# pzimbrod/fem-glass-tempering

Measured on AMD Instinct MI355X. Metric: DOF-updates/sec (coupled thermo-visco time step, 3D CG1 hex), higher is better.
Workload: dtype f64; 1 GPU; C4 3D plate CG1/CG1 400x400x50 hex (8200851 T-dofs), dt 0.1, coupled 6-term Prony; parallelism=single GPU, one partition (no communication), output=none (reference writes VTX/XDMF every step), krylov_form=PETSc KSPCG, geometric-multigrid V-cycle preconditioner, preconditioner=gmg, visco_fields=state (T, Tf, Tf_partial, phi, xi, s_tilde, sigma_tilde, sigma)

## Files before the change

fem-glass-tempering_amd/csrc/tv_cg.hip:

```cpp
#include <algorithm>
#include <cstdlib>

#include "tv_stencil.h"


#include <cstdio>
#include <vector>

namespace tv {
namespace {


using buf_t = __amdgpu_buffer_rsrc_t;
using b64v = unsigned int __attribute__((ext_vector_type(2)));
constexpr uint32_t kBadOff = 0x40000000u;
__device__ __forceinline__ buf_t mk_rsrc(const void* p, uint32_t bytes) {
  const uint64_t a = (uint64_t)p;
  const uint32_t lo = __builtin_amdgcn_readfirstlane((uint32_t)a);
  const uint32_t hi = __builtin_amdgcn_readfirstlane((uint32_t)(a >> 32));
  void* q = (void*)(((uint64_t)hi << 32) | lo);
  return __builtin_amdgcn_make_buffer_rsrc(q, (short)0, (int)__builtin_amdgcn_readfirstlane(bytes), 0x00020000);
}
__device__ __forceinline__ double bload(buf_t r, uint32_t off) {
  return __builtin_bit_cast(double, __builtin_amdgcn_raw_buffer_load_b64(r, (int)off, 0, 0));
// ... 771 lines not shown
    const double us_p = My0 * x0 + My1 * x1 + My2 * x2;
    const double vs_p = Ky0 * x0 + Ky1 * x1 + Ky2 * x2;
    double um_p = us_p;
    if (MODE == MODE_RES) um_p = My0 * lds[NA - 1][buf][wave][lane] + My1 * vm + My2 * lds[NA - 1][buf][wave + 2][lane];
    const double t_p = um_p + da * vs_p;
    if (L >= q0 + 1 && L <= q1) {
      const int q = L - 1;
      const double2* cq = cql[q - q0 + 1];
      const double2 c01 = cq[0], c23 = cq[1], c45 = cq[2], c67 = cq[3], c89 = cq[4];
      const double S1 = c01.x * t_m + c01.y * t_c + c23.x * t_p + (c23.y * us_m + c45.x * us_c + c45.y * us_p);
      const double S2 = c67.x * us_m + c67.y * us_c + c89.x * us_p;
      const double2 xlo = cxl[0][lane], xdi = cxl[1][lane], xup = cxl[2][lane];
      const double Lt = xup.x * S1 + xup.y * S2;
      const double Rt = xlo.x * S1 + xlo.y * S2;
      const double y = (xdi.x * S1 + xdi.y * S2) + (shr1(Lt) + shl1(Rt));
      const bool q_owned = (raxis == 2) ? true : (q >= kb && q < ke);
      const bool q_inwin = (raxis == 2) ? true : (q >= wb && q < we);
      const bool wr = writer && row_ok && row_owned && q_owned;
      const bool inwin = row_inwin && q_inwin;
      double yb = y;
      if (fq0 && q == 0) yb += yq0;
      if (fq1 && q == nQ - 1) yb += yq1;
      if (POST) {
        const double xm = xdi.x, xk = xdi.y;
        const double dI = xm * My1 * c01.y + ((xk * My1 * c67.y + xm * Ky1 * c67.y) + xm * My1 * c45.x);
        const double dq = (bnd_lr || bnd_q(q)) ? pd : 1.0 / dI;
        const double zq = xc + pa.omega * dq * (pr - yb);
        bstore(rso, inwin ? vo_wr + plane_off(q) : kBadOff, zq);
        zz += wr ? zq * zq : 0.0;
        zr += wr ? zq * pr : 0.0;
      } else {
        bstore(rso, inwin ? vo_wr + plane_off(q) : kBadOff, yb);
      }
      if (MODE == MODE_JAC && !POST) dot += wr ? xc * yb : 0.0;
    }
    xc = x1;
    us_m = us_c; us_c = us_p;
    t_m = t_c; t_c = t_p;
  };
  for (int L = q0 - 1; L <= q1; L += PF + 1) {
#pragma unroll
    for (int s = 0; s <= PF; ++s) {
      const int sf = (s + PF) % (PF + 1);
      fetch(vo_own, L + s + PF, ra0[sf], ra1[sf]);
      fetch(vo_halo, L + s + PF, rh0[sf], rh1[sf]);
      fetch_post(L + s + PF, rr[sf], rd[sf]);
      step(L + s, ra0[s], ra1[s], rh0[s], rh1[s], POST ? rr[s] : 0.0, POST ? rd[s] : 0.0);
    }
  }
  if (POST) {
    zz = wave_sum(zz);
    zr = wave_sum(zr);
    if (lane == 0) {
      red[wave] = zz;
      fsm[wave] = zr;
    }
    __syncthreads();
    if (threadIdx.x == 0) {
      double a = 0.0, c = 0.0;
#pragma unroll
      for (int w = 0; w < R; ++w) {
        a += red[w];
        c += fsm[w];
      }
      store_partial(&partials[2 * (int64_t)bid], a);
      store_partial(&partials[2 * (int64_t)bid + 1], c);
    }
    return;
  }
  if (MODE == MODE_JAC && partials != nullptr) {
    dot = wave_sum(dot);
    if (lane == 0) red[wave] = dot;
    __syncthreads();
    if (threadIdx.x == 0) {
      double s = 0.0;
#pragma unroll
      for (int w = 0; w < R; ++w) s += red[w];
      store_partial(&partials[blockIdx.x], s);
    }
    fused_reduce_tail<1>(rt, nrec);
  }
}


__device__ __forceinline__ uint32_t ff_off_x(const CgGrid& g, int i, int j, int k) {
  const int f = (i == 0) ? 0 : (i == g.n0 - 1 ? 1 : -1);
  if (f < 0 || g.ffoff[f] < 0) return kBadOff;
  return (uint32_t)(g.ffoff[f] + j + (int64_t)g.n1 * k) * 8u;
}
__device__ __forceinline__ uint32_t ff_off_r(const CgGrid& g, int ra, int i, int j, int k) {
  const int c = (ra == 1) ? j : k, n = (ra == 1) ? g.n1 : g.n2;
  const int side = (c == 0) ? 0 : (c == n - 1 ? 1 : -1);
  if (side < 0 || i < 0 || i >= g.n0) return kBadOff;
  const int f = 2 * ra + side;
  if (g.ffoff[f] < 0) return kBadOff;
  return (uint32_t)(g.ffoff[f] + i + (int64_t)g.n0 * ((ra == 1) ? k : j)) * 8u;
}

struct CgsScal {
  double a, b;
  bool first;
};

template <bool INIT>
__device__ __forceinline__ void cgs_node(const CgsScal& k, double R, double S, double W, double D, double ff,
                                         double& s, double& r, double& u) {
  if (INIT) {
    s = 0.0;
    r = R;
  } else {
    const double wf = W + ff;
    s = k.first ? wf : wf + k.b * S;
    r = R - k.a * s;
  }
  u = D * r;
}

template <bool INIT, int R>
__device__ void face_block_cgs(const CgGrid& g, const CgsBuffers& v, const CgsScal& ks, int raxis,
                               double* __restrict__ partials, int fb, const FaceOff& fo, double* sm,
                               double (*red)[R]) {
  double (*sT)[kWave] = reinterpret_cast<double (*)[kWave]>(sm);
  double (*sP)[kWave] = reinterpret_cast<double (*)[kWave]>(sm + (R + 1) * kWave);
  double (*sCD)[R][kWave] = reinterpret_cast<double (*)[R][kWave]>(sm + 2 * (R + 1) * kWave);
  int f = 0;
  while (f < 5 && fb >= fo.off[f + 1]) ++f;
  const int a = f >> 1, side = f & 1;
  const int t1 = (a == 0) ? 1 : 0, t2 = (a == 2) ? 1 : 2;
  const int n[3] = {g.n0, g.n1, g.n2};
  const int n1 = n[t1], n2 = n[t2];
  const int nseg1 = (n1 + kSeg - 1) / kSeg;
  const int tile = fb - fo.off[f];
  const int seg = tile % nseg1, tb = tile / nseg1;
  const int lane = threadIdx.x & (kWave - 1);
  const int wave = __builtin_amdgcn_readfirstlane(threadIdx.x >> 6);
  const int c1 = seg * kSeg - 1 + lane;
  const int r0 = tb * (R - 1);
  const bool ok1 = c1 >= 0 && c1 < n1;
  const buf_t rsFin = mk_rsrc(v.fin, (uint32_t)(g.ffsize * 8));
  struct Stg {
    double tt, R_, D, S, W, fx, fr;
    bool ok;
  };
  auto stage_ld = [&](int cc2) -> Stg {
    Stg q{};
    q.ok = ok1 && cc2 >= 0 && cc2 < n2;
    int c[3];
    c[t1] = q.ok ? c1 : 0;
    c[t2] = q.ok ? cc2 : 0;
    c[a] = side ? n[a] - 1 : 0;
    const int64_t o = c[0] + (int64_t)g.n0 * c[1] + (int64_t)g.n0 * g.n1 * c[2];
    q.tt = v.T[o];
    q.R_ = v.rin[o];
    q.D = v.dinv[o];
    if (!INIT) {
      q.S = ks.first ? 0.0 : v.sin[o];
      q.W = v.win[o];
      q.fx = bload(rsFin, ff_off_x(g, c[0], c[1], c[2]));
      q.fr = bload(rsFin, ff_off_r(g, raxis, c[0], c[1], c[2]));
    }
    return q;
  };
  auto stage_st = [&](int row, const Stg& q) {
    double s, r, u;
    cgs_node<INIT>(ks, q.R_, q.S, q.W, q.D, INIT ? 0.0 : q.fx + q.fr, s, r, u);
    sT[row][lane] = q.ok ? q.tt : 0.0;
// ... 392 lines not shown
    const int nn[3] = {g.n0, g.n1, g.n2};
    double acc = 0.0;
#pragma unroll 1
    for (int a = 0; a < 3; ++a) {
      if ((c[a] == 0 && g.bnd[a][0]) || (c[a] == nn[a] - 1 && g.bnd[a][1]))
        acc += facet_direct<MODE, false>(g, i, j, k, a, T, x, nullptr, 0.0, true);
    }
    out[n] += acc;
    if (MODE == MODE_JAC) dot += x[n] * acc;
    if (MODE == MODE_RES && dinv != nullptr) dinv[n] = 1.0 / diag_value<3, true>(g, T, n);
  }
  if (MODE == MODE_JAC && partials != nullptr) {
    dot = wave_sum(dot);
    const int lane = threadIdx.x & 63, wave = threadIdx.x >> 6;
    if (lane == 0) red[wave] = dot;
    __syncthreads();
    if (threadIdx.x == 0) store_partial(&partials[blockIdx.x], (red[0] + red[1]) + (red[2] + red[3]));
  }
}


int dim_of(const CgGrid& g) { return g.deg2 ? 1 : (g.deg1 ? 2 : 3); }

constexpr int kMarchMinBlocks = 1024;
constexpr int kMarchMinQ = 6;
constexpr int kMarchSmallTiles = 256;

struct Launch {
  int blocks, nseg, kfirst, nplanes, wmode, rows;
  int nparts;
  bool march;
  int raxis, qchunk;
};

bool use_march(const CgGrid& g) {
  const int64_t bytes = (int64_t)g.n0 * g.n1 * g.n2 * 8;
  return dim_of(g) == 3 && bytes < (int64_t)kBadOff;
}

int bnd_blocks(const CgGrid& g) {
  int64_t b = (g.n_bnodes + kBlock - 1) / kBlock;
  return (int)std::max<int64_t>(1, std::min<int64_t>(b, 1024));
}

Launch plan(const CgGrid& g, bool ghosts) {
  Launch L{};
  L.nseg = (g.n0 + kSeg - 1) / kSeg;
  L.march = use_march(g);
  if (L.march) {
    L.raxis = (g.n2 >= g.n1) ? 2 : 1;
    L.rows = kRows;
    const int nR = (L.raxis == 1) ? g.n1 : g.n2;
    const int nQ = (L.raxis == 1) ? g.n2 : g.n1;
    const int nrb = (nR + L.rows - 1) / L.rows;
    int nchunks = 1;
    while ((int64_t)L.nseg * nrb * nchunks < kMarchMinBlocks && nQ / (nchunks * 2) >= kMarchMinQ) nchunks *= 2;
    while ((int64_t)L.nseg * nrb * nchunks < kMarchSmallTiles && nQ / (nchunks * 2) >= 2) nchunks *= 2;
    while ((nQ + nchunks - 1) / nchunks > kFaceChunk) ++nchunks;
    L.qchunk = (nQ + nchunks - 1) / nchunks;
    nchunks = (nQ + L.qchunk - 1) / L.qchunk;
    L.blocks = L.nseg * nrb * nchunks;
    L.nparts = L.blocks + face_offsets(g, L.rows, 3 - L.raxis).off[6];
    return L;
  }
  L.kfirst = ghosts ? g.k_begin - g.g_lo : g.k_begin;
  L.nplanes = (g.k_end - g.k_begin) + (ghosts ? g.g_lo + g.g_hi : 0);
  L.wmode = (g.n1 >= 4) ? 0 : 1;
  if (L.wmode == 0) {
    L.blocks = L.nseg * ((g.n1 + 3) / 4) * L.nplanes;
  } else {
    const int64_t waves = (int64_t)L.nseg * g.n1 * L.nplanes;
    L.blocks = (int)((waves + 3) / 4);
  }
  L.nparts = L.blocks;
  return L;
}

template <int MODE, bool FUSEP>
bool launch_rows(const CgGrid& g, const double* T, const double* in0, const double* in1, double* out,
                 double* pout, const PcgState* st, double* partials, bool ghosts, hipStream_t s,
                 const RedTail* tail = nullptr, int it_host = 0, bool addfaces = true, double* dinv_bnd = nullptr) {
  const Launch L = plan(g, ghosts);
  if (L.blocks <= 0) return false;
  if (L.march) {
    const bool folded = MODE == MODE_JAC;
    RedTail rt{};
    if (folded && tail && partials) rt = *tail;
    const FaceOff fo = folded ? face_offsets(g, L.rows, 3 - L.raxis) : FaceOff{};
    const int grid = L.blocks + fo.off[6];
    hipLaunchKernelGGL((k_cg_march<MODE, FUSEP, kRows, 1, 2>), dim3(grid), dim3(kRows * kWave), 0, s, g, T, in0, in1,
                       out, pout, st, partials, L.nseg, L.raxis, L.qchunk, rt, L.nparts, L.blocks, fo, it_host,
                       PostArgs{});
    if (folded && !FUSEP && addfaces && fo.off[6] > 0) {
      const int64_t nodes = 2 * ((int64_t)g.n1 * (g.w_end - g.w_begin) + (int64_t)g.n0 * std::max(g.n1, g.n2));
      const int nb = (int)std::max<int64_t>(1, std::min<int64_t>((nodes + kBlock - 1) / kBlock, 1024));
      hipLaunchKernelGGL(k_cg_addfaces, dim3(nb), dim3(kBlock), 0, s, g, out, L.raxis, st);
    }
    if (folded) return rt.counter != nullptr;
    if (g.n_bnodes > 0) {
      hipLaunchKernelGGL((k_cg_boundary<MODE, FUSEP>), dim3(bnd_blocks(g)), dim3(kBlock), 0, s, g, g.bnodes,
                         g.n_bnodes, T, FUSEP ? in1 : in0, pout, out, st,
                         partials ? partials + L.blocks : nullptr, dinv_bnd);
    }
    return false;
  }
  switch (dim_of(g)) {
    case 1:
      hipLaunchKernelGGL((k_cg_rows<1, MODE, FUSEP>), dim3(L.blocks), dim3(kBlock), 0, s, g, T, in0, in1, out,
                         pout, st, partials, L.nseg, L.kfirst, L.nplanes, L.wmode);
      break;
    case 2:
      hipLaunchKernelGGL((k_cg_rows<2, MODE, FUSEP>), dim3(L.blocks), dim3(kBlock), 0, s, g, T, in0, in1, out,
                         pout, st, partials, L.nseg, L.kfirst, L.nplanes, L.wmode);
      break;
    default:
      hipLaunchKernelGGL((k_cg_rows<3, MODE, FUSEP>), dim3(L.blocks), dim3(kBlock), 0, s, g, T, in0, in1, out,
                         pout, st, partials, L.nseg, L.kfirst, L.nplanes, L.wmode);
  }
  return false;
}

__global__ __launch_bounds__(kBlock) void k_mg_post_faces(FaceAdd fa, int raxis, const double* __restrict__ r,
                                                         const double* __restrict__ dinv, double omega,
                                                         double* __restrict__ z, double* __restrict__ partials,
                                                         int rec0, RedTail rt, const PcgState* __restrict__ st, int kb,
                                                         int ke, int wb, int we) {
  if (st->done) return;
  const int n0 = fa.n0, n1 = fa.n1, n2 = fa.n2;
  const int64_t nA = 2 * (int64_t)n1 * n2;
  const int nO = (raxis == 2) ? n1 : n2;
  const int64_t nB = 2 * (int64_t)(n0 - 2) * nO;
  double a0 = 0.0, a1 = 0.0;
  const FaceRsrc fr = face_rsrc(fa);
  for (int64_t t = blockIdx.x * (int64_t)kBlock + threadIdx.x; t < nA + nB; t += (int64_t)gridDim.x * kBlock) {
    int i, j, k;
    if (t < nA) {
      const int64_t pl = (int64_t)n1 * n2;
      const int side = (int)(t / pl);
      const int64_t e = t - side * pl;
      i = side ? n0 - 1 : 0;
      j = (int)(e % n1);
      k = (int)(e / n1);
    } else {
      const int64_t u = t - nA, pl = (int64_t)(n0 - 2) * nO;
      const int side = (int)(u / pl);
      const int64_t e = u - side * pl;
      i = 1 + (int)(e % (n0 - 2));
      const int o = (int)(e / (n0 - 2));
      if (raxis == 2) {
        j = o;
        k = side ? n2 - 1 : 0;
      } else {
        k = o;
        j = side ? n1 - 1 : 0;
      }
    }
    if (k < wb || k >= we) continue;
    const int64_t q = i + (int64_t)n0 * (j + (int64_t)n1 * k);
    const double zo = z[q], dq = dinv[q], rq = r[q];
    const double add = face_at_nb(fa, fr, i, j, k);
    const double zn = zo - omega * dq * add;
    z[q] = zn;
    if (k < kb || k >= ke) continue;
    a0 += zn * zn - zo * zo;
    a1 += (zn - zo) * rq;
  }
// ... 4 lines not shown
  if (lane == 0) {
    red[0][wave] = a0;
    red[1][wave] = a1;
  }
  __syncthreads();
  if (threadIdx.x < 2) {
    const int w = threadIdx.x;
    store_partial(&partials[2 * ((int64_t)rec0 + blockIdx.x) + w], (red[w][0] + red[w][1]) + (red[w][2] + red[w][3]));
  }
  fused_reduce_tail<2>(rt, rec0 + (int)gridDim.x);
}

__global__ __launch_bounds__(kBlock) void k_mg_prep_inject(MgPrep p) {
  const int64_t t = blockIdx.x * (int64_t)kBlock + threadIdx.x;
  int l = 0;
  while (l + 1 < p.nlev && t >= p.off_n[l + 1]) ++l;
  l = __builtin_amdgcn_readfirstlane(l);
  const MgXfer& x = p.xf[l];
  const int64_t e = t - p.off_n[l];
  const int64_t nc = (int64_t)x.cn[0] * x.cn[1] * x.cn[2];
  if (e >= nc) return;
  int c0 = (int)(e % x.cn[0]);
  int c1 = (int)((e / x.cn[0]) % x.cn[1]);
  int c2 = (int)(e / ((int64_t)x.cn[0] * x.cn[1]));
  for (int m = l; m >= 0; --m) {
    const MgXfer& y = p.xf[m];
    c0 = y.ri[0][3 * c0 + 1];
    c1 = y.ri[1][3 * c1 + 1];
    c2 = y.ri[2][3 * c2 + 1];
  }
  const MgXfer& b = p.xf[0];
  p.T[l][e] = p.Tbase[c0 + (int64_t)b.fn[0] * (c1 + (int64_t)b.fn[1] * c2)];
}

__global__ __launch_bounds__(kBlock) void k_mg_prep_diag(MgPrep p) {
  const int64_t t = blockIdx.x * (int64_t)kBlock + threadIdx.x;
  int l = 0;
  while (l + 1 < p.nlev && t >= p.off_b[l + 1]) ++l;
  l = __builtin_amdgcn_readfirstlane(l);
  const CgGrid& g = p.g[l];
  const int64_t e = t - p.off_b[l];
  if (e >= g.n_bnodes) return;
  const int64_t n = g.bnodes[e];
  p.dinv[l][n] = 1.0 / diag_value<3, true>(g, p.T[l], n);
}


template <int R>
__global__ __launch_bounds__(R * kWave) void k_cg_faces_all(CgGrid g, const double* __restrict__ T,
                                                            const double* __restrict__ x, FaceOff fo,
                                                            const PcgState* __restrict__ st) {
  if (st != nullptr && st->done) return;
  __shared__ double fsm[(8 * R + 8) * kWave];
  __shared__ double red[R];
  face_block<false, R>(g, T, x, x, x, 0.0, nullptr, RedTail{}, 0, (int)blockIdx.x, fo, fsm, red, 0);
}

}

int launch_cg_japply_post(const CgGrid& g, const double* T, const double* x, const double* r, const double* dinv,
                          double omega, double* z, const PcgState* st, double* partials, const RedTail* tail,
                          hipStream_t s) {
  const Launch L = plan(g, false);
  if (!L.march || g.n0 < 3) return -1;
  const FaceOff fo = face_offsets(g, L.rows, 3 - L.raxis);
  const int grid = L.blocks + fo.off[6];
  const PostArgs pa{r, dinv, omega};
  hipLaunchKernelGGL((k_cg_march<MODE_JAC, false, 8, 1, 2, true>), dim3(grid), dim3(8 * kWave), 0, s, g, T, x,
                     nullptr, z, nullptr, st, partials, L.nseg, L.raxis, L.qchunk, RedTail{}, L.nparts, L.blocks, fo,
                     0, pa);
  const FaceAdd fa = cg_face_add(g, 0);
  const int nO = (L.raxis == 2) ? g.n1 : g.n2;
  const int64_t nodes = 2 * (int64_t)g.n1 * g.n2 + 2 * (int64_t)(g.n0 - 2) * nO;
  constexpr int cap = 240;
  const int nb = (int)std::max<int64_t>(1, std::min<int64_t>((nodes + kBlock - 1) / kBlock, cap));
  const RedTail rt = tail ? *tail : RedTail{};
  hipLaunchKernelGGL(k_mg_post_faces, dim3(nb), dim3(kBlock), 0, s, fa, L.raxis, r, dinv, omega, z, partials,
                     L.blocks, rt, st, g.k_begin, g.k_end, g.w_begin, g.w_end);
  return L.blocks + nb;
}

bool cg_uses_march(const CgGrid& g) { return use_march(g); }

void launch_mg_prepare(const MgPrep& p, hipStream_t s) {
  const int64_t nn = p.off_n[p.nlev], nb = p.off_b[p.nlev];
  if (nn > 0) hipLaunchKernelGGL(k_mg_prep_inject, dim3((unsigned)((nn + kBlock - 1) / kBlock)), dim3(kBlock), 0, s, p);
  if (nb > 0) hipLaunchKernelGGL(k_mg_prep_diag, dim3((unsigned)((nb + kBlock - 1) / kBlock)), dim3(kBlock), 0, s, p);
}

int cg_num_blocks(const CgGrid& g, bool with_ghost_planes) { return plan(g, with_ghost_planes).nparts; }

FaceAdd cg_face_add(const CgGrid& g, int64_t t_off) {
  FaceAdd fa{};
  if (!use_march(g)) return fa;
  fa.on = 1;
  fa.n0 = g.n0;
  fa.n1 = g.n1;
  fa.n2 = g.n2;
  fa.t_off = t_off;
  fa.inv_n0 = 1.0 / g.n0;
  fa.inv_plane = 1.0 / ((double)g.n0 * g.n1);
  const int qaxis = 3 - plan(g, true).raxis;
  for (int f = 0; f < 6; ++f) fa.ff[f] = ((f >> 1) == qaxis) ? nullptr : g.fface[f];
  return fa;
}

void launch_cg_residual(const CgGrid& g, const double* T, const double* Tp, double* F, hipStream_t s) {
  launch_rows<MODE_RES, false>(g, T, T, Tp, F, nullptr, nullptr, nullptr, false, s);
}

bool launch_cg_residual_diag(const CgGrid& g, const double* T, const double* Tp, double* F, double* dinv,
                             hipStream_t s) {
  if (!use_march(g) || !g.bnodes || g.n_bnodes <= 0) return false;
  launch_rows<MODE_RES, false>(g, T, T, Tp, F, nullptr, nullptr, nullptr, false, s, nullptr, 0, true, dinv);
  return true;
}

void launch_cg_japply(const CgGrid& g, const double* T, const double* x, double* y, double* partials,
                      int* n_partials, hipStream_t s, const PcgState* st) {
  launch_rows<MODE_JAC, false>(g, T, x, nullptr, y, nullptr, st, partials, false, s);
  if (n_partials) *n_partials = plan(g, false).nparts;
}

bool launch_cg_japply_tail(const CgGrid& g, const double* T, const double* x, double* y, const PcgState* st,
                           double* partials, const RedTail* tail, hipStream_t s) {
  return launch_rows<MODE_JAC, false>(g, T, x, nullptr, y, nullptr, st, partials, false, s, tail, 0, true);
}

void launch_cg_facet_faces(const CgGrid& g, const double* T, const double* x, const PcgState* st, hipStream_t s) {
  const FaceOff fo = face_offsets(g, kRows, -1);
  if (fo.off[6] <= 0) return;
  hipLaunchKernelGGL(k_cg_faces_all<kRows>, dim3(fo.off[6]), dim3(kRows * kWave), 0, s, g, T, x, fo, st);
}

FaceAdd cg_face_add_all(const CgGrid& g) {
  FaceAdd fa = cg_face_add(g, 0);
  if (!fa.on) return fa;
  for (int f = 0; f < 6; ++f) fa.ff[f] = g.fface[f];
  return fa;
}

void launch_cg_japply_partial(const CgGrid& g, const double* T, const double* x, double* y, const PcgState* st,
                              hipStream_t s) {
  launch_rows<MODE_JAC, false>(g, T, x, nullptr, y, nullptr, st, nullptr, false, s, nullptr, 0, false);
}

bool launch_cg_japply_fused(const CgGrid& g, const double* T, const double* z, double* pA, double* pB,
                            double* w, const PcgState* st, double* partials, int* n_partials,
                            hipStream_t s, const RedTail* tail, int it_host) {
  if (tail && tail->lag && tail->lag_kind != 3) return false;
  const bool fused = launch_rows<MODE_JAC, true>(g, T, z, pA, w, pB, st, partials, true, s, tail, it_host);
  if (n_partials) *n_partials = plan(g, true).nparts;
  return fused;
}

bool launch_cg_cgs(const CgGrid& g, bool init, const CgsBuffers& v, PcgState* st, double* partials,
                   hipStream_t s, const RedTail* tail, int it_host, const double* lag_sums) {
  if (!use_march(g)) return false;
  const Launch L = plan(g, true);
  const FaceOff fo = face_offsets(g, L.rows, 3 - L.raxis);
  const int grid = L.blocks + fo.off[6];
  RedTail rt{};
  if (tail) rt = *tail;
  if (init)
    hipLaunchKernelGGL((k_cgs_march<true, 8, 1>), dim3(grid), dim3(8 * kWave), 0, s, g, v, st, partials, L.nseg,
                       L.raxis, L.qchunk, rt, grid, L.blocks, fo, it_host, lag_sums);
// ... 32 lines not shown
```

fem-glass-tempering_amd/csrc/tv_context.cpp:

```cpp
#include <cstdlib>

#include "tv_ctx.h"

namespace tv {

static std::mutex g_err_mu;
static std::string g_err;

void set_global_error(const std::string& m) {
  std::lock_guard<std::mutex> lk(g_err_mu);
  g_err = m;
}

void axis_coefs(const std::vector<double>& X, int first, int count, std::vector<double>& out) {
  const int n = (int)X.size();
  out.assign((size_t)count * C_NCOEF, 0.0);
  for (int q = 0; q < count; ++q) {
    const int i = first + q;
    double* c = &out[(size_t)q * C_NCOEF];
    if (n == 1) {
      c[C_MDI] = 1.0;
      continue;
    }
    const double hlo = (i > 0) ? X[i] - X[i - 1] : 0.0;
// ... 41 lines not shown
    perm[0] = 0; perm[1] = -1; perm[2] = -1;
  } else if (d == 2) {
    perm[0] = 0; perm[1] = -1; perm[2] = 1;
  } else {
    int pa = m->part_axis;
    if (pa < 0) pa = (m->n_cells[1] >= m->n_cells[2]) ? 1 : 2;
    if (pa != 1 && pa != 2) return false;
    perm[0] = 0; perm[2] = pa; perm[1] = (pa == 1) ? 2 : 1;
  }
  return true;
}

void part_planes(int N2, int P, int p, int* b0, int* b1) {
  *b0 = (int)((int64_t)N2 * p / P);
  *b1 = (int)((int64_t)N2 * (p + 1) / P);
}

int build_cg_grid(Ctx* c, int d, const std::vector<double> (&X)[3], int first2, int n2, int g_lo, int g_hi,
                         bool bnd2lo, bool bnd2hi, CgGrid& g, double** coef, int64_t** bnodes, double** ffbuf) {
  g.n0 = (int)X[0].size();
  g.n1 = (int)X[1].size();
  g.g_lo = g_lo;
  g.g_hi = g_hi;
  g.n2 = n2;
  g.k_begin = g_lo;
  g.k_end = n2 - g_hi;
  g.w_begin = g.k_begin - std::max(0, g_lo - 1);
  g.w_end = g.k_end + std::max(0, g_hi - 1);
  g.deg1 = X[1].size() == 1;
  g.deg2 = X[2].size() == 1;
  g.bnd[0][0] = g.bnd[0][1] = 1;
  g.bnd[1][0] = g.bnd[1][1] = g.deg1 ? 0 : 1;
  g.bnd[2][0] = (!g.deg2 && bnd2lo) ? 1 : 0;
  g.bnd[2][1] = (!g.deg2 && bnd2hi) ? 1 : 0;
  const int first[3] = {0, 0, first2};
  const int cnt[3] = {g.n0, g.n1, g.n2};
  for (int s = 0; s < 3; ++s) {
    std::vector<double> cf;
    axis_coefs(X[s], first[s], cnt[s], cf);
    HIPC(hipMalloc(&coef[s], cf.size() * sizeof(double)));
    HIPC(hipMemcpy(coef[s], cf.data(), cf.size() * sizeof(double), hipMemcpyHostToDevice));
    g.coef[s] = coef[s];
  }
  const int64_t plane = (int64_t)g.n0 * g.n1;
  for (int f = 0; f < 6; ++f) g.ffoff[f] = -1;
  if (d == 3) {
    std::vector<int64_t> bn;
    for (int k = g.w_begin; k < g.w_end; ++k)
      for (int j = 0; j < g.n1; ++j)
        for (int i = 0; i < g.n0; ++i) {
          const bool on = (i == 0 && g.bnd[0][0]) || (i == g.n0 - 1 && g.bnd[0][1]) ||
                          (j == 0 && g.bnd[1][0]) || (j == g.n1 - 1 && g.bnd[1][1]) ||
                          (k == 0 && g.bnd[2][0]) || (k == g.n2 - 1 && g.bnd[2][1]);
          if (on) bn.push_back((int64_t)i + (int64_t)g.n0 * j + plane * k);
        }
    if (!bn.empty()) {
      HIPC(hipMalloc(bnodes, bn.size() * sizeof(int64_t)));
      HIPC(hipMemcpy(*bnodes, bn.data(), bn.size() * sizeof(int64_t), hipMemcpyHostToDevice));
    }
    g.bnodes = *bnodes;
    g.n_bnodes = (int64_t)bn.size();
    const int nn[3] = {g.n0, g.n1, g.n2};
    int64_t tot = 0;
    for (int f = 0; f < 6; ++f) {
      const int ax = f >> 1, side = f & 1;
      g.fface[f] = nullptr;
      g.fn1[f] = g.fn2[f] = 0;
      g.ffoff[f] = -1;
      if (!g.bnd[ax][side]) continue;
      const int t1 = (ax == 0) ? 1 : 0, t2 = (ax == 2) ? 1 : 2;
      g.fn1[f] = nn[t1];
      g.fn2[f] = nn[t2];
      g.ffoff[f] = tot;
      tot += (int64_t)nn[t1] * nn[t2];
    }
    g.ffsize = tot;
    for (int q = 0; q < 2; ++q) {
      HIPC(hipMalloc(&ffbuf[q], sizeof(double) * (size_t)std::max<int64_t>(1, tot)));
      HIPC(hipMemsetAsync(ffbuf[q], 0, sizeof(double) * (size_t)std::max<int64_t>(1, tot), c->stream));
      g.ffbuf[q] = ffbuf[q];
    }
    for (int f = 0; f < 6; ++f) g.fface[f] = (g.ffoff[f] >= 0) ? ffbuf[0] + g.ffoff[f] : nullptr;
  }
  return TV_OK;
}

int setup_mixed_part(Ctx* c) {
  const int d = c->dim, nl = 1 << d;
  const int P = c->n_parts, p = c->part;
  const bool last = (p == P - 1);
  const int b0 = c->plane_begin, b1 = c->plane_end;
  const int C[3] = {std::max(1, c->Ncell_glob[0]), std::max(1, c->Ncell_glob[1]), std::max(1, c->Ncell_glob[2])};
  const int N0 = c->Nnode_glob[0], N1 = c->Nnode_glob[1];
  const bool act[3] = {true, c->perm[1] >= 0, c->perm[2] >= 0};
  const int64_t npl = (int64_t)N0 * N1;
  const int64_t pc = (int64_t)C[0] * C[1];
  auto corner = [&](const int bits[3]) {
    int l = 0, k = 0;
    for (int s = 0; s < 3; ++s) {
      if (!act[s]) continue;
      l |= bits[s] << k;
      ++k;
    }
    return l;
  };
  std::vector<int> map;
  if (c->fam_T == TV_DG) {
    c->mixed_part = 1;
    const int nq = b1 - b0 + 1;
    c->nS = npl * nq;
    c->ownS_off = 0;
    c->ownS_n = npl * (last ? nq : nq - 1);
    c->globS_off = npl * b0;
    c->outS_n = c->nS;
    c->outT_n = c->ownT_n;
    const DgGrid& g = c->dg;
    map.assign((size_t)c->nS, -1);
    for (int k = b0; k <= b1; ++k)
      for (int j = 0; j < N1; ++j)
        for (int i = 0; i < N0; ++i) {
          const int ci[3] = {std::min(i, C[0] - 1), act[1] ? std::min(j, C[1] - 1) : 0,
                             act[2] ? std::min(k, C[2] - 1) : 0};
          const int bits[3] = {i - ci[0], j - ci[1], k - ci[2]};
          const int l = corner(bits);
          const int kl = ci[2] - b0 + g.k_begin;
          int64_t base, stride;
          if (kl < g.k_begin) base = g.gofs[0], stride = pc;
          else if (kl >= g.k_end) base = g.gofs[1], stride = pc;
          else base = (int64_t)(kl - g.k_begin) * pc, stride = g.own;
          if (base < 0) return c->fail(TV_ERR_ARG, "mixed partition: a sigma node outside the local cells (internal)");
          const int64_t dof = base + (int64_t)l * stride + ci[0] + (int64_t)C[0] * ci[1];
          map[(size_t)(i + N0 * (j + (int64_t)N1 * (k - b0)))] = (int)dof;
        }
  } else {
    c->mixed_part = 2;
    const int L1 = std::min(b1, C[2]);
    const int64_t ncl = pc * (L1 - b0);
    c->nS = ncl * nl;
    c->ownS_off = 0;
    c->ownS_n = c->nS;
    c->globS_off = pc * nl * b0;
    c->outS_n = c->nS;
    const CgGrid& g = c->cg;
    c->outT_n = c->ownT_n + (g.g_hi ? npl : 0);
    map.assign((size_t)c->nS, -1);
    for (int64_t cl = 0; cl < ncl; ++cl) {
      const int ci[3] = {(int)(cl % C[0]), (int)((cl / C[0]) % C[1]), b0 + (int)(cl / pc)};
      for (int l = 0; l < nl; ++l) {
        int bits[3] = {0, 0, 0}, k = 0;
        for (int s = 0; s < 3; ++s) {
          if (!act[s]) continue;
          bits[s] = (l >> k) & 1;
          ++k;
        }
        const int kl = ci[2] + bits[2] - (b0 - g.g_lo);
        if (kl < 0 || kl >= g.n2) return c->fail(TV_ERR_ARG, "mixed partition: a corner outside the local planes (internal)");
        map[(size_t)((int64_t)l * ncl + cl)] =
            (int)((ci[0] + bits[0]) + (int64_t)g.n0 * ((ci[1] + bits[1]) + (int64_t)g.n1 * kl));
      }
    }
  }
  HIPC(hipMalloc(&c->map, sizeof(int) * (size_t)std::max<int64_t>(1, c->nS)));
  HIPC(hipMemcpy(c->map, map.data(), sizeof(int) * (size_t)c->nS, hipMemcpyHostToDevice));
  return TV_OK;
}

// ... 975 lines not shown
```

fem-glass-tempering_amd/csrc/tv_internal.h:

```cpp
#pragma once
#include <hip/hip_runtime.h>
#include <cstdint>
#include <string>
#include <vector>

#include "tvfem.h"

namespace tv {

constexpr int kWave = 64;
constexpr int kSeg = kWave - 2;
constexpr int kBlock = 256;

enum { C_MLO = 0, C_MDI, C_MUP, C_KLO, C_KDI, C_KUP, C_HLO, C_HHI, C_NCOEF };

struct PostArgs {
  const double* r;
  const double* dinv;
  double omega;
};

constexpr int kDeepGhosts = 3;

struct CgGrid {
  int n0, n1, n2;
  int k_begin, k_end;
  int g_lo, g_hi;
  int w_begin, w_end;
  int deg1, deg2;
  int bnd[3][2];
  const double* coef[3];
  double dt, dt_alpha, dt_f;
  double a_rad, a_conv;
  double T_amb, T_amb4;
  const int64_t* bnodes;
  int64_t n_bnodes;
  double* fface[6];
  int fn1[6], fn2[6];
  double* ffbuf[2];
  int64_t ffoff[6];
  int64_t ffsize;
};

struct DgGrid {
  int c0, c1, c2;
  int k_begin, k_end;
  int deg1, deg2;
  int bnd[3][2];
  const double* h[3];
  const double* ih[3];
  double hdiam_inv;
  double dt, dt_alpha, dt_f;
  double a_rad, a_conv;
  double T_amb, T_amb4;
  double penalty;
  int tile, tile_chunk;
  int64_t own;
  int64_t gofs[2];
};

constexpr int kShards = 8;
constexpr int kTailCounters = kShards + 1;
constexpr int kCounterWords = 32;
constexpr int kUpdateCounter = 2 * kTailCounters;
static_assert(kUpdateCounter < kCounterWords, "counter words");

struct PcgState {
  double beta, betaold, dpi, dpiold, a, dp, rnorm0, ttol;
  double rtol, atol, dtol;
  int it, done, reason, max_it;
  int post;
  int accept_its;
  int relaxed;
  double dx_norm2;
  double a_prev;
  double gamma, eta;
};

struct RedTail {
  unsigned* counter;
  const double* partials;
  double* out;
  PcgState* st;
  int kind;
  uint64_t* ts;
  const double* lag = nullptr;
  int lag_kind = 0;
};

enum PcgReason {
  R_RUNNING = 0,
  R_CONV_RTOL = 2, R_CONV_ATOL = 3,
  R_DIV_ITS = -3, R_DIV_DTOL = -4, R_DIV_INDEF_PC = -8, R_DIV_NANINF = -9, R_DIV_INDEF_MAT = -10,
  R_SKIPPED = -100,
};

struct ViscoConst {
  double H_over_Rg, inv_Tb, dt, half_dt, alpha_s, dalpha, inv_dim;
  double lambda_m[6], m_n[6], lambda_g[6], g_n[6], lambda_k[6], k_n[6];
  double chi;
  int paper;
};

struct NewtonGate {
  const double* flag = nullptr;
};
#ifdef __HIPCC__
__device__ __forceinline__ bool newton_gate_open(const NewtonGate& g) {
  return g.flag == nullptr || *g.flag != 0.0;
}
#endif

struct ViscoFields {
  int64_t n;
  int64_t off_T, off_S;
  int64_t sT, sS;
  const int* map;
  double* T; double* Tp; double* Tn; double* phi; double* phin; double* xi;
  double* Tf; double* Tfp;
  double* th; double* tot; double* dev;
  double* ds; double* dsig;
  double* st; double* sgt;
  double* sp; double* sgp;
  double* sigma;
  double* Tfo;
  int copy_Tprev;
  int* tflag;
  NewtonGate gate;
};

struct UmGrid {
  int dim;
  int64_t nv, nc, nf, nslice;
  int64_t nrow;
  const int64_t* soff;
  const int* cols;
  const double* V;
  const double* M;
  const double* K;
  const double* bvec;
  const double* vdiag;
  const double* V14;
  double* J14;
  const double* M14;
  const double* K14;
  const int64_t* brow;
  int64_t nbr;
  int64_t s1, s2;
  const int* fv;
  const double* fw;
  const int* boff;
  const int* binc;
  double dt, dt_alpha, dt_f;
  double a_rad, a_conv;
  double T_amb, T_amb4;
};

struct Sell {
  int64_t nrow = 0, ncol = 0, nslice = 0;
  const int64_t* soff = nullptr;
  const int* cols = nullptr;
  const void* vals = nullptr;
  const int* perm = nullptr;
  int csr = 0, fp32 = 0;
};
int amg_num_blocks(const Sell& M);
void launch_amg_apply(const Sell& A, const PcgState* st, const double* x, double* y, hipStream_t s);
void launch_amg_restrict(const Sell& R, const PcgState* st, const double* x, const double* x2, const double* dinv_c,
                         double omega_c, double* b_c, double* x_c, hipStream_t s);
void launch_amg_prolong(const Sell& P, const PcgState* st, const double* x_c, const double* x_old, double* x_new,
                        hipStream_t s);
void launch_amg_post(const Sell& A, const PcgState* st, const double* x, const double* b, const double* dinv,
                     double omega, double* y, hipStream_t s);
int launch_amg_prolong0(const Sell& P, const PcgState* st, const double* x_c, const double* x0, const double* r,
                        double* z, double* partials, const RedTail* tail, hipStream_t s);
Sell um_operator(const UmGrid& g);

struct UmDevice;
int um_setup(int dim, int64_t nv, int64_t nrow, const double* xyz, int64_t nc, const int64_t* cells, UmGrid& g,
             UmDevice*& dev, hipStream_t s, std::string& err);
void launch_um_pack(const int64_t* idx, int64_t n, const double* v, double* out, hipStream_t s);
void um_free(UmDevice* dev);
int64_t um_boundary_vertices(const UmDevice* dev, std::vector<unsigned char>& mask);
int64_t um_nnz(const UmDevice* dev);
int um_num_blocks(const UmGrid& g);
int um_rcb(int dim, int64_t nv, const double* xyz, int64_t nc, const int64_t* cells, int n_parts, int* part,
           std::string& err);
void launch_um_residual(const UmGrid& g, const double* T, const double* Tp, double* F, hipStream_t s);
void launch_um_japply(const UmGrid& g, const double* T, const double* x, double* y, hipStream_t s);
void launch_geo_restrict0(const int64_t (&fn)[3], const int64_t (&cn)[3], const PcgState* st, const double* r,
                          const double* dinv_c, double omega_c, double* b_c, double* x_c, hipStream_t s);
int launch_geo_prolong0(const int64_t (&fn)[3], const int64_t (&cn)[3], const PcgState* st, const double* x_c,
                        const double* x0, const double* r, double* z, double* partials, const RedTail* tail,
                        hipStream_t s);
void launch_sg_apply(const UmGrid& g, const PcgState* st, const double* x, const double* b, const double* dinv,
                     double omega, double* y, hipStream_t s);
void launch_um_robin_fold(const UmGrid& g, const double* T, hipStream_t s);
void launch_um_diag(const UmGrid& g, const double* T, double* d, int invert, hipStream_t s);
int launch_um_japply_fused(const UmGrid& g, const double* T, const double* z, double* pA, double* pB, double* w,
                           const PcgState* st, double* partials, int it_host, const RedTail* tail, hipStream_t s);

void launch_cg_residual(const CgGrid& g, const double* T, const double* Tp, double* F, hipStream_t s);
bool launch_cg_residual_diag(const CgGrid& g, const double* T, const double* Tp, double* F, double* dinv,
                             hipStream_t s);
void launch_cg_japply(const CgGrid& g, const double* T, const double* x, double* y, double* partials,
                      int* n_partials, hipStream_t s, const PcgState* st = nullptr);
bool launch_cg_japply_fused(const CgGrid& g, const double* T, const double* z, double* pA, double* pB,
                            double* w, const PcgState* st, double* partials, int* n_partials,
                            hipStream_t s, const RedTail* tail = nullptr, int it_host = 0);
struct CgsBuffers {
  const double* T;
  const double* rin;
  double* rout;
  const double* sin;
  double* sout;
  const double* win;
  double* wout;
  const double* fin;
  double* fout;
  double* p;
  double* x;
  const double* dinv;
};

bool launch_cg_cgs(const CgGrid& g, bool init, const CgsBuffers& v, PcgState* st, double* partials,
                   hipStream_t s, const RedTail* tail, int it_host, const double* lag_sums);
int cg_cgs_records(const CgGrid& g);
bool cg_cgs_supported(const CgGrid& g);
void launch_cg_diag(const CgGrid& g, const double* T, double* dinv, int invert, hipStream_t s, bool bnd_only = false);
int cg_num_blocks(const CgGrid& g, bool with_ghost_planes);

void launch_dg_residual(const DgGrid& g, const double* T, const double* Tp, double* F, hipStream_t s);
void launch_dg_japply(const DgGrid& g, const double* T, const double* x, double* y, double* partials,
                      int* n_partials, hipStream_t s, const PcgState* st = nullptr);
bool launch_dg_japply_fused(const DgGrid& g, const double* T, const double* z, double* pA, double* pB,
                            double* w, const PcgState* st, double* partials, int* n_partials,
                            hipStream_t s, const RedTail* tail = nullptr);
void launch_dg_diag(const DgGrid& g, const double* T, double* dinv, int invert, hipStream_t s);
int dg_num_blocks(const DgGrid& g);
int64_t dg_gface_size(const DgGrid& g);
void launch_dg_gface(const DgGrid& g, const double* T, double* gface, hipStream_t s);
void launch_dg_bsmooth(const DgGrid& g, const PcgState* st, const double* b, const double* w, const double* gface,
                       double omega, double* x, int mode, hipStream_t s);
void launch_dg_bupdate(const DgGrid& g, const PcgState* st, const double* pA, const double* pB, const double* w,
                       const double* gface, double omega, double* r, double* dx, double* x0, int it_host, int init,
                       hipStream_t s);
int launch_dg_bpost(const DgGrid& g, const PcgState* st, const double* x0, const double* r, const double* w,
                    const double* gface, double omega, double* z, double* partials, const RedTail* tail, hipStream_t s);

void launch_visco(int dim, int all, const ViscoConst& c, const ViscoFields& f, hipStream_t s);
void launch_visco_Tpass(int dim, int all, const ViscoConst& c, const ViscoFields& f, hipStream_t s);
void launch_visco_Spass(int dim, int all, const ViscoConst& c, const ViscoFields& f, hipStream_t s);

constexpr int kVecBlocks = 1024;
constexpr int kVecBlocksMin = 256;
constexpr int kVecNodesPerThread = 16;
constexpr int kVecBlocksMax = 8192;
void launch_pcg_init(int64_t n, const double* r, const double* dinv, double* z, double* dx,
                     double* partials, hipStream_t s);
struct FaceAdd {
  int on;
  int n0, n1, n2;
  int64_t t_off;
  double inv_n0, inv_plane;
  const double* ff[6];
};
FaceAdd cg_face_add(const CgGrid& g, int64_t t_off);


struct MgXfer {
  int fn[3], cn[3];
  int coarse[3];
  int f_kb, f_ke, c_kb, c_ke;
  const int* pi[3];
  const double* pw[3];
  const int* ri[3];
  const double* rw[3];
  int aligned;
};
void launch_mg_restrict(const MgXfer& x, const PcgState* st, const double* bf, const double* wf, const FaceAdd* fa,
                        const double* mask, double* bc, const double* dinv_c, double omega_c, double* xc,
                        hipStream_t s);
struct RRAxis {
  const int* f0;
  const double* w;
};
struct RRArgs {
// ... 102 lines not shown
```

Before: 850.3 million DOF-updates/s.

## Add direct non-marching Jacobian-apply kernel for small CG grids

Adds a k_cg_direct kernel that computes the CG1 hex Jacobian apply by loading a 3-row by (NQ+2)-plane neighbourhood per wave into registers, instead of marching along an axis. It is used only for JAC mode without partials or reductions, and only when the grid has fewer than 500k nodes (overridable by env var), so it mainly targets the coarse multigrid levels. The aim is more parallelism and shorter dependency chains on small grids where the marching kernel has too few blocks. The cost is redundant plane loads at chunk boundaries.

```diff
diff --git a/fem-glass-tempering_amd/csrc/tv_cg.hip b/fem-glass-tempering_amd/csrc/tv_cg.hip
--- a/fem-glass-tempering_amd/csrc/tv_cg.hip
+++ b/fem-glass-tempering_amd/csrc/tv_cg.hip
@@ -877,6 +877,144 @@
   }
 }
 
+using b128v = unsigned int __attribute__((ext_vector_type(4)));
+using d2v = double __attribute__((ext_vector_type(2)));
+__device__ __forceinline__ d2v bload2(buf_t r, uint32_t off) {
+  return __builtin_bit_cast(d2v, __builtin_amdgcn_raw_buffer_load_b128(r, (int)off, 0, 0));
+}
+
+constexpr int kDirectQ = 2;
+
+template <int NQ, int R>
+__global__ __launch_bounds__(R * kWave) void k_cg_direct(CgGrid g, const double* __restrict__ T,
+                                                         const double* __restrict__ x, double* __restrict__ out,
+                                                         const PcgState* __restrict__ st, int nseg, int raxis,
+                                                         int nmain, FaceOff fo) {
+  __shared__ double fsm[(4 * R + 2) * kWave];
+  __shared__ double red[R];
+  const int bid = (int)blockIdx.x;
+  if (bid >= nmain) {
+    if (st != nullptr && st->done) return;
+    face_block<false, R>(g, T, x, x, x, 0.0, nullptr, RedTail{}, 0, bid - nmain, fo, fsm, red, 0);
+    return;
+  }
+  const int lane = threadIdx.x & (kWave - 1);
+  const int wave = __builtin_amdgcn_readfirstlane(threadIdx.x >> 6);
+  const int n0 = g.n0;
+  const int nR = (raxis == 1) ? g.n1 : g.n2;
+  const int nQ = (raxis == 1) ? g.n2 : g.n1;
+  const uint32_t sR = (raxis == 1) ? (uint32_t)n0 : (uint32_t)n0 * (uint32_t)g.n1;
+  const uint32_t sQ = (raxis == 1) ? (uint32_t)n0 * (uint32_t)g.n1 : (uint32_t)n0;
+  const int nqc = (nQ + NQ - 1) / NQ;
+  int t = (bid & 7) * (nmain >> 3) + min(bid & 7, nmain & 7) + (bid >> 3);
+  const int per = nseg * nqc;
+  const int rb = t / per;
+  t -= rb * per;
+  const int seg = t % nseg, qc = t / nseg;
+  const int r = rb * R + wave;
+  if (r >= nR) return;
+  const int q0 = qc * NQ;
+  const int i = seg * kSeg - 1 + lane;
+  const bool col_ok = (i >= 0) && (i < n0);
+  const bool writer = col_ok && lane >= 1 && lane <= kSeg;
+  const double* coefR = (raxis == 1) ? g.coef[1] : g.coef[2];
+  const double* coefQ = (raxis == 1) ? g.coef[2] : g.coef[1];
+  const int bq_lo = (raxis == 1) ? g.bnd[2][0] : g.bnd[1][0];
+  const int bq_hi = (raxis == 1) ? g.bnd[2][1] : g.bnd[1][1];
+  const bool fq0 = q0 == 0 && bq_lo;
+  const bool fq1 = nQ - 1 >= q0 && nQ - 1 < q0 + NQ && bq_hi;
+  const bool fq = fq0 || fq1;
+  const int qf = fq0 ? 0 : nQ - 1;
+  const uint32_t nbytes = (uint32_t)g.n0 * (uint32_t)g.n1 * (uint32_t)g.n2 * 8u;
+  const buf_t rsX = mk_rsrc(x, nbytes);
+  const buf_t rsO = mk_rsrc(out, nbytes);
+  const buf_t rsT = mk_rsrc(T, fq ? nbytes : 0u);
+  const buf_t rsS = mk_rsrc(st, st != nullptr ? (uint32_t)sizeof(PcgState) : 0u);
+  const buf_t rsC = mk_rsrc(g.coef[0], (uint32_t)n0 * (uint32_t)(C_NCOEF * 8));
+  uint32_t vo[3];
+#pragma unroll
+  for (int b = 0; b < 3; ++b) {
+    const int rr = r + b - 1;
+    vo[b] = (col_ok && rr >= 0 && rr < nR) ? ((uint32_t)i + sR * (uint32_t)rr) * 8u : kBadOff;
+  }
+  auto plane_off = [&](int L) -> uint32_t { return (L >= 0 && L < nQ) ? (sQ * (uint32_t)L) * 8u : kBadOff; };
+  const uint32_t so = (lane - kWave >= n0) ? 4u : 0u;
+  const int done_v = __builtin_amdgcn_raw_buffer_load_b32(rsS, (int)(so + (uint32_t)offsetof(PcgState, done)), 0, 0);
+  double X[3][NQ + 2];
+#pragma unroll
+  for (int p = 0; p < NQ + 2; ++p) {
+    const uint32_t po = plane_off(q0 - 1 + p);
+#pragma unroll
+    for (int b = 0; b < 3; ++b) X[b][p] = bload(rsX, vo[b] + po);
+  }
+  const uint32_t co = col_ok ? (uint32_t)i * (uint32_t)(C_NCOEF * 8) : kBadOff;
+  const d2v cA = bload2(rsC, co), cB = bload2(rsC, co + 16u), cC = bload2(rsC, co + 32u), cD = bload2(rsC, co + 48u);
+  double Tf[3];
+#pragma unroll
+  for (int b = 0; b < 3; ++b) Tf[b] = bload(rsT, vo[b] + plane_off(qf));
+  const double* cr = coefR + (int64_t)r * C_NCOEF;
+  const double My0 = kld(cr, C_MLO), My1 = kld(cr, C_MDI), My2 = kld(cr, C_MUP);
+  const double Ky0 = kld(cr, C_KLO), Ky1 = kld(cr, C_KDI), Ky2 = kld(cr, C_KUP);
+  const double hq_own = kld(cr, C_HHI);
+  const double hq_lowv = kld(coefR + (int64_t)(r >= 1 ? r - 1 : 0) * C_NCOEF, C_HHI);
+  const double hq_low = (r >= 1) ? hq_lowv : 0.0;
+  double Mz[NQ][3], Kz[NQ][3];
+#pragma unroll
+  for (int p = 0; p < NQ; ++p) {
+    const double* cq = coefQ + (int64_t)min(q0 + p, nQ - 1) * C_NCOEF;
+    Mz[p][0] = kld(cq, C_MLO); Mz[p][1] = kld(cq, C_MDI); Mz[p][2] = kld(cq, C_MUP);
+    Kz[p][0] = kld(cq, C_KLO); Kz[p][1] = kld(cq, C_KDI); Kz[p][2] = kld(cq, C_KUP);
+  }
+  const double da = g.dt_alpha;
+
+  double yqf = 0.0;
+  if (fq) {
+    const bool cok = i >= 0 && i < n0 - 1;
+    const double h1 = cD.y;
+    double P[3];
+#pragma unroll
+    for (int b = 0; b < 3; ++b) {
+      P[b] = X[b][1];
+#pragma unroll
+      for (int p = 2; p <= NQ; ++p) P[b] = (qf - q0 + 1 == p) ? X[b][p] : P[b];
+    }
+    double ya, yb, yc, yd;
+    facet_corners(g, cok && r < nR - 1, h1, hq_own, Tf[1], Tf[2], P[1], P[2], ya, yb, yc, yd);
+    yqf = ya + shr1(yb);
+    facet_corners(g, cok && r >= 1, h1, hq_low, Tf[0], Tf[1], P[0], P[1], ya, yb, yc, yd);
+    yqf += yc + shr1(yd);
+  }
+
+  double us[NQ + 2], tt[NQ + 2];
+#pragma unroll
+  for (int p = 0; p < NQ + 2; ++p) {
+    const double x0 = X[0][p], x1 = X[1][p], x2 = X[2][p];
+    const double us_p = My0 * x0 + My1 * x1 + My2 * x2;
+    const double vs_p = Ky0 * x0 + Ky1 * x1 + Ky2 * x2;
+    us[p] = us_p;
+    tt[p] = us_p + da * vs_p;
+  }
+  const int wb = g.w_begin, we = g.w_end;
+  const bool row_inwin = (raxis == 2) ? (r >= wb && r < we) : true;
+#pragma unroll
+  for (int p = 0; p < NQ; ++p) {
+    const int q = q0 + p;
+    const double t_m = tt[p], t_c = tt[p + 1], t_p = tt[p + 2];
+    const double us_m = us[p], us_c = us[p + 1], us_p = us[p + 2];
+    const double k0 = da * Kz[p][0], k1 = da * Kz[p][1], k2 = da * Kz[p][2];
+    const double m0 = da * Mz[p][0], m1 = da * Mz[p][1], m2 = da * Mz[p][2];
+    const double S1 = Mz[p][0] * t_m + Mz[p][1] * t_c + Mz[p][2] * t_p + (k0 * us_m + k1 * us_c + k2 * us_p);
+    const double S2 = m0 * us_m + m1 * us_c + m2 * us_p;
+    const double Lt = cB.x * S1 + cC.y * S2;
+    const double Rt = cA.x * S1 + cB.y * S2;
+    const double y = (cA.y * S1 + cC.x * S2) + (shr1(Lt) + shl1(Rt));
+    double yb = y;
+    if (fq && q == qf) yb += yqf;
+    const bool q_inwin = (raxis == 2) ? true : (q >= wb && q < we);
+    bstore(rsO, (writer && row_inwin && q_inwin && done_v == 0) ? vo[1] + plane_off(q) : kBadOff, yb);
+  }
+}
+
 
 __device__ __forceinline__ uint32_t ff_off_x(const CgGrid& g, int i, int j, int k) {
   const int f = (i == 0) ? 0 : (i == g.n0 - 1 ? 1 : -1);
@@ -1435,6 +1573,21 @@
                  const RedTail* tail = nullptr, int it_host = 0, bool addfaces = true, double* dinv_bnd = nullptr) {
   const Launch L = plan(g, ghosts);
   if (L.blocks <= 0) return false;
+  if constexpr (MODE == MODE_JAC && !FUSEP) {
+    const int nR = (L.raxis == 1) ? g.n1 : g.n2, nQ = (L.raxis == 1) ? g.n2 : g.n1;
+    if (L.march && g.direct && partials == nullptr && tail == nullptr && nQ > kDirectQ) {
+      const FaceOff fo = face_offsets(g, kRows, 3 - L.raxis);
+      const int nmain = L.nseg * ((nR + kRows - 1) / kRows) * ((nQ + kDirectQ - 1) / kDirectQ);
+      hipLaunchKernelGGL((k_cg_direct<kDirectQ, kRows>), dim3(nmain + fo.off[6]), dim3(kRows * kWave), 0, s, g, T,
+                         in0, out, st, L.nseg, L.raxis, nmain, fo);
+      if (addfaces && fo.off[6] > 0) {
+        const int64_t nodes = 2 * ((int64_t)g.n1 * (g.w_end - g.w_begin) + (int64_t)g.n0 * std::max(g.n1, g.n2));
+        const int nb = (int)std::max<int64_t>(1, std::min<int64_t>((nodes + kBlock - 1) / kBlock, 1024));
+        hipLaunchKernelGGL(k_cg_addfaces, dim3(nb), dim3(kBlock), 0, s, g, out, L.raxis, st);
+      }
+      return false;
+    }
+  }
   if (L.march) {
     const bool folded = MODE == MODE_JAC;
     RedTail rt{};
@@ -1605,6 +1758,14 @@
 
 bool cg_uses_march(const CgGrid& g) { return use_march(g); }
 
+constexpr int64_t kDirectMaxNodes = 500000;
+bool cg_direct_wanted(const CgGrid& g) {
+  if (!use_march(g)) return false;
+  int64_t lim = kDirectMaxNodes;
+  if (const char* e = std::getenv("TVFEM_CG_DIRECT")) lim = std::strtoll(e, nullptr, 0);
+  return (int64_t)g.n0 * g.n1 * g.n2 < lim;
+}
+
 void launch_mg_prepare(const MgPrep& p, hipStream_t s) {
   const int64_t nn = p.off_n[p.nlev], nb = p.off_b[p.nlev];
   if (nn > 0) hipLaunchKernelGGL(k_mg_prep_inject, dim3((unsigned)((nn + kBlock - 1) / kBlock)), dim3(kBlock), 0, s, p);
diff --git a/fem-glass-tempering_amd/csrc/tv_context.cpp b/fem-glass-tempering_amd/csrc/tv_context.cpp
--- a/fem-glass-tempering_amd/csrc/tv_context.cpp
+++ b/fem-glass-tempering_amd/csrc/tv_context.cpp
@@ -147,6 +147,7 @@
     }
     for (int f = 0; f < 6; ++f) g.fface[f] = (g.ffoff[f] >= 0) ? ffbuf[0] + g.ffoff[f] : nullptr;
   }
+  g.direct = (d == 3 && cg_direct_wanted(g)) ? 1 : 0;
   return TV_OK;
 }
 
diff --git a/fem-glass-tempering_amd/csrc/tv_internal.h b/fem-glass-tempering_amd/csrc/tv_internal.h
--- a/fem-glass-tempering_amd/csrc/tv_internal.h
+++ b/fem-glass-tempering_amd/csrc/tv_internal.h
@@ -40,6 +40,7 @@
   double* ffbuf[2];
   int64_t ffoff[6];
   int64_t ffsize;
+  int direct;
 };
 
 struct DgGrid {
@@ -203,6 +204,7 @@
 void launch_cg_residual(const CgGrid& g, const double* T, const double* Tp, double* F, hipStream_t s);
 bool launch_cg_residual_diag(const CgGrid& g, const double* T, const double* Tp, double* F, double* dinv,
                              hipStream_t s);
+bool cg_direct_wanted(const CgGrid& g);
 void launch_cg_japply(const CgGrid& g, const double* T, const double* x, double* y, double* partials,
                       int* n_partials, hipStream_t s, const PcgState* st = nullptr);
 bool launch_cg_japply_fused(const CgGrid& g, const double* T, const double* z, double* pA, double* pB,
```

After: 856.3 million DOF-updates/s, median of 6. Within noise of the previous version (+0.7%).
